# lixilinx/psgd_tf

Measured on AMD Instinct MI355X. Metric: uvd_update_apply_params_per_sec, higher is better.
Workload: dtype f32

## Files before the change

### psgd_tf_amd/csrc/psgd_uvd.hip

```cpp
#include "uvd_kernels.h"
#include "psgd_hip.h"
#include <math.h>

namespace psgd {

const UvdOps* uvd_ops_group0(int r);
const UvdOps* uvd_ops_group1(int r);
const UvdOps* uvd_ops_group2(int r);
const UvdOps* uvd_ops_group3(int r);

const UvdWideOps* uvd_wide_group0(int r);
const UvdWideOps* uvd_wide_group1(int r);
const UvdWideOps* uvd_wide_group2(int r);
const UvdWideOps* uvd_wide_group3(int r);
const UvdWideOps* uvd_wide_ops_for_rank(int r) {
  if (r <= PSGD_UVD_MAX_RANK || r > 2 * PSGD_UVD_MAX_RANK) return nullptr;
  switch ((r - 33) / 8) {
    case 0: return uvd_wide_group0(r);
    case 1: return uvd_wide_group1(r);
    case 2: return uvd_wide_group2(r);
    default: return uvd_wide_group3(r);
  }
}

// ... 44 lines not shown

static int ws_open(void* ws, int64_t ws_bytes, int64_t N, int r, Ws* out) {
  if (N <= 0) return PSGD_ERR_BAD_ARG;
  if (r < 1 || r > PSGD_UVD_MAX_RANK) return PSGD_ERR_RANK;
  if (!ws || (reinterpret_cast<uintptr_t>(ws) & 255)) return PSGD_ERR_WORKSPACE;
  const WsLayout L = ws_layout(N, r);
  if (ws_bytes < L.total) return PSGD_ERR_WORKSPACE;
  char* b = static_cast<char*>(ws);
  out->sums = reinterpret_cast<double*>(b + L.sums_off);
  out->coef = reinterpret_cast<float*>(b + L.coef_off);
  out->maxbuf = reinterpret_cast<float*>(b + L.max_off);
  out->part = b + L.part_off;
  out->pmax = reinterpret_cast<float*>(b + L.pmax_off);
  out->nabla = reinterpret_cast<float*>(b + L.nabla_off);
  return PSGD_OK;
}

static inline bool misaligned16(const void* p) { return (reinterpret_cast<uintptr_t>(p) & 15) != 0; }

static int g_tune_staging = 0;
static int g_tune_blocks_per_cu = 0;
static int g_tune_tiles_per_wave = 8;

constexpr int kProfSlots = 8;
constexpr int kProfMaxPairs = 4096;
struct ProfPair { hipEvent_t e0, e1; };
static int g_prof_on = 0;
static ProfPair g_prof_pairs[kProfSlots][kProfMaxPairs];
static int g_prof_created[kProfSlots];
static int g_prof_used[kProfSlots];

struct ProfScope {
  hipEvent_t e1 = nullptr;
  hipStream_t st;
  ProfScope(int slot, hipStream_t s) : st(s) {
    if (!g_prof_on || slot < 0 || slot >= kProfSlots || g_prof_used[slot] >= kProfMaxPairs) return;
    const int i = g_prof_used[slot];
    if (i >= g_prof_created[slot]) {
      if (hipEventCreate(&g_prof_pairs[slot][i].e0) != hipSuccess) return;
      if (hipEventCreate(&g_prof_pairs[slot][i].e1) != hipSuccess) return;
      g_prof_created[slot] = i + 1;
    }
    g_prof_used[slot] = i + 1;
    (void)hipEventRecord(g_prof_pairs[slot][i].e0, st);
    e1 = g_prof_pairs[slot][i].e1;
  }
  ~ProfScope() {
    if (e1) (void)hipEventRecord(e1, st);
  }
};

static int num_cus() {
  static int n = 0;
  if (n == 0) {
    int dev = 0;
    (void)hipGetDevice(&dev);
    int v = 0;
    if (hipDeviceGetAttribute(&v, hipDeviceAttributeMultiprocessorCount, dev) != hipSuccess || v <= 0) v = 256;
    n = v;
  }
  return n;
}

static inline int use_nt(int64_t N, int r) {
  if (g_tune_staging == 1) return 0;
  if (g_tune_staging == 2) return 1;
  return (int64_t)N * r * 8 > (int64_t)192 * 1024 * 1024;
}

int policy_nt(int64_t stream_bytes) {
  if (g_tune_staging == 1) return 0;
  if (g_tune_staging == 2) return 1;
  return stream_bytes > (int64_t)192 * 1024 * 1024;
}
int policy_grid_blocks(int occ) {
  if (occ <= 0) occ = 1;
  if (g_tune_blocks_per_cu > 0 && g_tune_blocks_per_cu < occ) occ = g_tune_blocks_per_cu;
  if (g_tune_blocks_per_cu < 0) occ = -g_tune_blocks_per_cu;
  return occ;
}
int device_cus() { return num_cus(); }

static int g_tune_grid[16] = {0};

static int sweep_grid(const UvdOps* ops, int r, int which, int64_t N, int hard_cap) {
  static int occ_cache[PSGD_UVD_MAX_RANK + 1][16];
  if (which >= 0 && which < 16 && g_tune_grid[which] > 0) {
    const int64_t tiles = (N + ops->tile_rows - 1) / ops->tile_rows;
    int64_t grid = (tiles + kWavesPerBlock - 1) / kWavesPerBlock;
    if (grid > g_tune_grid[which]) grid = g_tune_grid[which];
    if (grid > hard_cap) grid = hard_cap;
    return (int)(grid < 1 ? 1 : grid);
  }
  int occ = occ_cache[r][which];
  if (occ == 0) {
    occ = ops->occupancy(which);
    if (occ <= 0) occ = 1;
    occ_cache[r][which] = occ;
  }
  if (which == kOccUpdS2U || which == kOccUpdS2V || which == kOccUpdS2F) {
    const int want = ((long)ops->tile_rows * r * 4 >= 4096) ? 1 : 2;
    if (want < occ) occ = want;
  } else if (which == kOccFinal) {
    occ = 1;
  }
  if (g_tune_blocks_per_cu > 0 && g_tune_blocks_per_cu < occ) occ = g_tune_blocks_per_cu;
  if (g_tune_blocks_per_cu < 0) occ = -g_tune_blocks_per_cu;
  const int64_t tiles = (N + ops->tile_rows - 1) / ops->tile_rows;
  int64_t grid = (tiles + kWavesPerBlock - 1) / kWavesPerBlock;
  int64_t cap = (int64_t)num_cus() * occ;
  if (g_tune_blocks_per_cu == 0) {
    int64_t want = tiles / (kWavesPerBlock * (g_tune_tiles_per_wave > 0 ? g_tune_tiles_per_wave : 1));
    if (want < num_cus()) want = num_cus();
    if (cap > want) cap = want;
  }
  if (grid > cap) grid = cap;
  if (grid > hard_cap) grid = hard_cap;
  if (grid < 1) grid = 1;
  return (int)grid;
}

template <class T>
__global__ __launch_bounds__(kThreads) void k_reduce_sum(const T* __restrict__ part, int G, int L,
                                                         double* __restrict__ sums, float* __restrict__ coef) {
  __shared__ double red[kWavesPerBlock][64];
  const int lane = threadIdx.x & 63, w = threadIdx.x >> 6;
  const int id = blockIdx.x * 64 + lane;
  double s = 0.0;
  if (id < L) {
    int b = w;
    for (; b + 7 * kWavesPerBlock < G; b += 8 * kWavesPerBlock) {
      T x[8];
#pragma unroll
      for (int u = 0; u < 8; ++u) x[u] = part[(long)(b + u * kWavesPerBlock) * L + id];
#pragma unroll
      for (int u = 0; u < 8; ++u) s += (double)x[u];
    }
    for (; b < G; b += kWavesPerBlock) s += (double)part[(long)b * L + id];
  }
  red[w][lane] = s;
  __syncthreads();
  if (w == 0 && id < L) {
    const double t = ((red[0][lane] + red[1][lane]) + red[2][lane]) + red[3][lane];
    sums[id] = t;
    if (coef) coef[id] = (float)t;
  }
}

__global__ __launch_bounds__(kThreads) void k_reduce_sum_t(const float* __restrict__ part, int G, int L,
                                                           double* __restrict__ sums, float* __restrict__ coef) {
  const int lane = threadIdx.x & 63;
  const int id = blockIdx.x * kWavesPerBlock + (threadIdx.x >> 6);
  if (id >= L) return;
  const float* p = part + (long)id * G;
  float x[kMaxGrid / 64];
#pragma unroll
  for (int u = 0; u < kMaxGrid / 64; ++u) x[u] = p[min(lane + 64 * u, G - 1)];
  double s = 0.0;
#pragma unroll
  for (int u = 0; u < kMaxGrid / 64; ++u) s += (lane + 64 * u < G) ? (double)x[u] : 0.0;
#pragma unroll
  for (int off = 32; off > 0; off >>= 1) s += __shfl_down(s, off, 64);
  if (lane == 0) {
    sums[id] = s;
    if (coef) coef[id] = (float)s;
  }
// ... 653 lines not shown
      for (int off = 32; off > 0; off >>= 1) sum += __shfl_down(sum, off, 64);
      if (lane == 0) { pqs[e] = sum; pq[e] = sum; }
    }
  } else {
    for (int e = tid; e < 4 * r; e += blockDim.x) pqs[e] = pq[e];
    if (tid == 0) mx = maxbuf[0];
  }
  const int nb = (2 * r + 2 + 15) / 16;
  auto Gm = [&](int a, int b) -> double {
    if constexpr (DENSE) return gram[a * (2 * r + 2) + b];
    if (a > b) { const int t = a; a = b; b = t; }
    const int bi = a >> 4, bj = b >> 4, i = a & 15, j = b & 15;
    const int p = bi * nb - (bi * (bi - 1)) / 2 + (bj - bi);
    return gram[p * 256 + (i & 3) * 64 + (((i >> 2) << 4) | j)];
  };
  const bool act = tid < r;
  if (act) {
    for (int j0 = 0; j0 < r; j0 += 8) {
      double t[8];
#pragma unroll
      for (int u = 0; u < 8; ++u) t[u] = Gm(tid, (j0 + u < r) ? j0 + u : 0);
#pragma unroll
      for (int u = 0; u < 8; ++u)
        if (j0 + u < r) A[tid][j0 + u] = t[u];
    }
    if (update_U) {
      const double mu = c64[4 * r], aa = c64[4 * r + 1], ab = c64[4 * r + 2], bb = c64[4 * r + 3];
      const double Ua = c64[tid], Ub = c64[r + tid], c1 = c64[2 * r + tid], c2 = c64[3 * r + tid];
      for (int j = 0; j < r; ++j) {
        const double Uaj = c64[j], Ubj = c64[r + j], c1j = c64[2 * r + j], c2j = c64[3 * r + j];
        A[tid][j] += -mu * (Ua * c1j + c1 * Uaj - Ub * c2j - c2 * Ubj) +
                     mu * mu * (aa * c1 * c1j - ab * (c1 * c2j + c2 * c1j) + bb * c2 * c2j);
      }
    }
  }
  __syncthreads();
  const double mud = (double)(step / (mx + tiny));
  if (act) s1n[tid] = pqs[r + tid] - mud * pqs[3 * r + tid];
  __syncthreads();
  if (act) {
    double s2 = pqs[tid] - mud * pqs[2 * r + tid];
    for (int k = 0; k < r; ++k) s2 += A[tid][k] * s1n[k];
    coef[tid] = (float)s1n[tid];
    coef[r + tid] = (float)s2;
    s_out[tid] = s1n[tid];
    s_out[r + tid] = s2;
  }
}

}

using namespace psgd;

#define PSGD_CHECK_LAUNCH(expr)                 \
  do {                                          \
    const int _e = (expr);                      \
    if (_e != 0) return PSGD_ERR_LAUNCH;        \
  } while (0)

static inline int last_launch() { return (int)hipGetLastError(); }

extern "C" {

int psgd_abi_version(void) { return PSGD_ABI_VERSION; }

const char* psgd_error_string(int code) {
  switch (code) {
    case PSGD_OK: return "ok";
    case PSGD_ERR_BAD_ARG: return "bad argument (null pointer or non-positive size)";
    case PSGD_ERR_RANK: return "rank of modification outside [1, 32]";
    case PSGD_ERR_WORKSPACE: return "workspace missing, too small or not 256-byte aligned";
    case PSGD_ERR_ALIGN: return "matrix pointer not 16-byte aligned";
    case PSGD_ERR_LAUNCH: return "HIP kernel launch failed";
    case PSGD_ERR_SHAPE: return "inconsistent or unsupported matrix shapes";
    default: return "unknown error";
  }
}

int psgd_set_tuning(int key, int value) {
  if (key == 0) { g_tune_staging = value; return PSGD_OK; }
  if (key == 1) { g_tune_blocks_per_cu = value; return PSGD_OK; }
  if (key == 2) { g_tune_coef = value; return PSGD_OK; }
  if (key == 3) { g_tune_tiles_per_wave = value; return PSGD_OK; }
  if (key >= 10 && key < 26) { g_tune_grid[key - 10] = value; return PSGD_OK; }
  return PSGD_ERR_BAD_ARG;
}

int psgd_prof_enable(int on) {
  g_prof_on = on ? 1 : 0;
  for (int s = 0; s < kProfSlots; ++s) g_prof_used[s] = 0;
  return PSGD_OK;
}

int psgd_prof_collect(int slot, double* total_ms, int* count) {
  if (slot < 0 || slot >= kProfSlots || !total_ms || !count) return PSGD_ERR_BAD_ARG;
  double tot = 0.0;
  int n = 0;
  for (int i = 0; i < g_prof_used[slot]; ++i) {
    float ms = 0.0f;
    if (hipEventSynchronize(g_prof_pairs[slot][i].e1) != hipSuccess) continue;
    if (hipEventElapsedTime(&ms, g_prof_pairs[slot][i].e0, g_prof_pairs[slot][i].e1) != hipSuccess) continue;
    tot += ms;
    ++n;
  }
  g_prof_used[slot] = 0;
  *total_ms = tot;
  *count = n;
  return PSGD_OK;
}

int64_t psgd_uvd_workspace_bytes(int64_t N, int r) {
  if (N <= 0) return PSGD_ERR_BAD_ARG;
  if (r < 1 || r > PSGD_UVD_MAX_RANK) return PSGD_ERR_RANK;
  return ws_layout(N, r).total;
}

int psgd_uvd_ws_region(int which, int stage, int64_t N, int r, int64_t* offset_bytes, int64_t* count) {
  if (!offset_bytes || !count || N <= 0) return PSGD_ERR_BAD_ARG;
  if (r < 1 || r > PSGD_UVD_MAX_RANK) return PSGD_ERR_RANK;
  const WsLayout L = ws_layout(N, r);
  const int nc = 2 * r + 2, nb = (nc + 15) / 16, np = nb * (nb + 1) / 2;
  if (which == PSGD_WS_SUMS_F64) {
    if (stage == 1) { *offset_bytes = L.sums_off; *count = r; return PSGD_OK; }
    if (stage == 2) { *offset_bytes = L.sums_off + (int64_t)r * 8; *count = r; return PSGD_OK; }
    if (stage == 11) { *offset_bytes = L.sums_off; *count = (int64_t)np * 256; return PSGD_OK; }
    if (stage == 13) { *offset_bytes = L.sums_off + (int64_t)kPqSumsOff * 8; *count = 4 * r; return PSGD_OK; }
  } else if (which == PSGD_WS_MAX_F32) {
    if (stage == 10) { *offset_bytes = L.max_off; *count = 2; return PSGD_OK; }
    if (stage == 12) { *offset_bytes = L.max_off + 8; *count = 1; return PSGD_OK; }
  } else if (which == PSGD_WS_SEND_F64) {
    if (stage == 1 || stage == 2 || stage == 11) return psgd_uvd_ws_region(PSGD_WS_SUMS_F64, stage, N, r, offset_bytes, count);
    if (stage == 10) { *offset_bytes = L.sums_off + (int64_t)kBalD64Off * 8; *count = 2; return PSGD_OK; }
    if (stage == 12) { *offset_bytes = L.sums_off + (int64_t)(kPqSumsOff + 4 * r) * 8; *count = 1; return PSGD_OK; }
    if (stage == 13) { *offset_bytes = L.sums_off + (int64_t)kPqSumsOff * 8; *count = 4 * r + 1; return PSGD_OK; }
  }
  return PSGD_ERR_BAD_ARG;
}

int psgd_uvd_fold_gathered_f64(int stage, const double* gathered, int world, int64_t N, int r, void* ws,
                               int64_t ws_bytes, void* stream) {
  if (!gathered || world < 1) return PSGD_ERR_BAD_ARG;
  Ws w;
  const int rc = ws_open(ws, ws_bytes, N, r, &w);
  if (rc) return rc;
  int64_t off = 0, count = 0;
  const int rr = psgd_uvd_ws_region(PSGD_WS_SEND_F64, stage, N, r, &off, &count);
  if (rr) return rr;
  double* dst = reinterpret_cast<double*>(static_cast<char*>(ws) + off);
  int nsum = (int)count;
  float* maxdst = nullptr;
  if (stage == 10) { nsum = 0; maxdst = w.maxbuf; }
  else if (stage == 12) { nsum = 0; maxdst = w.maxbuf + 2; }
  else if (stage == 13) { nsum = 4 * r; maxdst = w.maxbuf + 2; }
  hipLaunchKernelGGL(k_fold_gathered, dim3(((int)count + 255) / 256), dim3(256), 0, static_cast<hipStream_t>(stream),
                     gathered, world, (int)count, nsum, dst, maxdst);
  PSGD_CHECK_LAUNCH(last_launch());
  return PSGD_OK;
}

int psgd_uvd_apply_sweep1_f32(const float* V, const float* d, const float* g, int64_t N, int r, void* ws,
                              int64_t ws_bytes, void* stream) {
  if (!V || !d || !g) return PSGD_ERR_BAD_ARG;
  Ws w;
  const int rc = ws_open(ws, ws_bytes, N, r, &w);
  if (rc) return rc;
  if (misaligned16(V)) return PSGD_ERR_ALIGN;
// ... 688 lines not shown
```

### psgd_tf_amd/csrc/uvd_kernels.h

```cpp
#pragma once
#include <hip/hip_runtime.h>
#include <stdint.h>
#include <type_traits>
#include "nanmax.h"

namespace psgd {

constexpr int kWave = 64;
constexpr int kWavesPerBlock = 4;
constexpr int kThreads = kWave * kWavesPerBlock;
constexpr int kMaxGrid = 2048;
constexpr int kGramMaxGrid = 1024;
#ifndef PSGD_TILE_CHUNK
#define PSGD_TILE_CHUNK 1
#endif
constexpr int kTileChunk = PSGD_TILE_CHUNK;

typedef float f32x4 __attribute__((ext_vector_type(4)));

#ifndef PSGD_WAVE_ID_VGPR
__device__ __forceinline__ int wave_in_block() { return __builtin_amdgcn_readfirstlane((int)(threadIdx.x >> 6)); }
#else
__device__ __forceinline__ int wave_in_block() { return (int)(threadIdx.x >> 6); }
#endif
// ... 862 lines not shown
    sweep_rows<R, 2, NV, (UPDATE_U ? 0 : 1), NT>(mats, vecs, UPDATE_U ? U : V, N, lds, body);
  }
  block_max_store(vmax, red, part_max + blockIdx.x);
}

template <int R, bool NT>
__global__ __launch_bounds__(kThreads) void k_uvd_final(const float* U, const float* V, float* d, const float* nabla,
                                                        const float* g, float* out, long N,
                                                        const float* __restrict__ coef, const float* __restrict__ maxbuf,
                                                        float step, float tiny) {
  __shared__ __attribute__((aligned(16))) float lds[kWavesPerBlock][sweep_lds_floats<R, 2, 3>()];
  const float mu = step / (maxbuf[0] + tiny);
  const float* const mats[2] = {U, V};
  const float* const vecs[3] = {d, nabla, g};
  sweep_rows<R, 2, 3, -1, NT>(mats, vecs, nullptr, N, lds[wave_in_block()],
                              [&](long row, bool valid, float (&x)[2][R], float (&s)[3]) {
                                const float dn = s[0] - (mu * s[0]) * s[1];
                                const float g1 = dn * s[2] + dot_row<R>(x[0], coef);
                                const float o = dn * (g1 + dot_row<R>(x[1], coef + R));
                                if (valid) {
                                  stream_store<NT>(d + row, dn);
                                  stream_store<NT>(out + row, o);
                                }
                              });
}

template <int R, bool NT, bool STR = false>
__global__ __launch_bounds__(kThreads) void k_rank2_update(float* M, const float* a, const float* b, long N,
                                                           const float* __restrict__ coef, long ld = R) {
  __shared__ __attribute__((aligned(16))) float lds[kWavesPerBlock][sweep_lds_floats<R, 1, 2>()];
  const float* const mats[1] = {M};
  const float* const vecs[2] = {a, b};
  sweep_rows<R, 1, 2, 0, NT, STR>(mats, vecs, M, N, lds[wave_in_block()],
                                  [&](long, bool, float (&x)[1][R], float (&s)[2]) {
#pragma unroll
                                    for (int c = 0; c < R; ++c) x[0][c] = x[0][c] - (s[0] * coef[c] - s[1] * coef[R + c]);
                                  }, NoTileHook(), RowStrides{{ld, ld}});
}

struct UvdOps {
  int tile_rows;
  int gram_len;
  int (*colreduce)(int nt, int nvec, const float* M, const float* a, const float* b, long N, float* part, int grid, hipStream_t st);
  int (*apply_s2)(int nt, const float* U, const float* d, const float* g, float* g1out, long N, const float* coef, float* part, int grid, hipStream_t st);
  int (*apply_s3)(int nt, const float* V, const float* d, float* out, long N, const float* coef, int grid, hipStream_t st);
  int (*rowdot_axpy)(int nt, const float* M, const float* x, float* out, long N, const float* coef, int grid, hipStream_t st);
  int (*update_gram)(int nt, const float* U, const float* V, const float* d, const float* v, const float* h, long N, double* part, int grid, hipStream_t st);
  int (*update_s2)(int nt, int update_U, float* U, float* V, const float* d, const float* v, const float* h, const float* g, long N, const float* coef, float* nabla, float* part_max, double* part_pq, int grid, hipStream_t st);
  int (*colreduce4)(int nt, const float* M, const float* const* x, long N, double* part, int grid, hipStream_t st);
  int (*rowdot_axpy4)(int nt, const float* M, const float* const* x, float* const* o, int ncols, long N, const float* coef, int grid, hipStream_t st);
  int (*rank2_update)(int nt, float* M, const float* a, const float* b, long N, const float* coef, int grid, hipStream_t st);
  int (*final_sweep)(int nt, const float* U, const float* V, float* d, const float* nabla, const float* g, float* out, long N, const float* coef, const float* maxbuf, float step, float tiny, int grid, hipStream_t st);
  int (*apply4_s1)(int nt, const float* V, const float* d, const float* const* x, long N, double* part, int grid, hipStream_t st);
  int (*apply4_s2)(int nt, const float* U, const float* d, const float* const* x, float* const* o, int ncols, long N, const float* coef, double* part, int grid, hipStream_t st);
  int (*apply4_s3)(int nt, const float* V, const float* d, float* const* o, int ncols, long N, const float* coef, int grid, hipStream_t st);
  int load_vec;
  int (*update_gram_ld)(const float* U, long ldU, const float* V, long ldV, const float* d, const float* v, const float* h, long N, double* part, int grid, hipStream_t st);
  int (*colreduce4_ld)(const float* M, long ld, const float* const* x, long N, double* part, int grid, hipStream_t st);
  int (*rowdot_axpy4_ld)(const float* M, long ld, const float* const* x, float* const* o, int ncols, long N, const float* coef, int grid, hipStream_t st);
  int (*rank2_update_ld)(float* M, long ld, const float* a, const float* b, long N, const float* coef, int grid, hipStream_t st);
  int (*occupancy)(int which);
};

struct UvdWideOps {
  int tile_rows;
  int (*colreduce4)(int nt, const float* M, const float* const* x, long N, double* part, int grid, hipStream_t st);
  int (*rowdot_axpy4)(int nt, const float* M, const float* const* x, float* const* o, int ncols, long N, const float* coef, int grid, hipStream_t st);
  int (*rank2_update)(int nt, float* M, const float* a, const float* b, long N, const float* coef, int grid, hipStream_t st);
  int (*apply4_s1)(int nt, const float* V, const float* d, const float* const* x, long N, double* part, int grid, hipStream_t st);
  int (*apply4_s2)(int nt, const float* U, const float* d, const float* const* x, float* const* o, int ncols, long N, const float* coef, double* part, int grid, hipStream_t st);
  int (*apply4_s3)(int nt, const float* V, const float* d, float* const* o, int ncols, long N, const float* coef, int grid, hipStream_t st);
  int (*update_s2)(int nt, int update_U, float* U, float* V, const float* d, const float* v, const float* h, const float* g, long N, const float* coef, float* nabla, float* part_max, double* part_pq, int grid, hipStream_t st);
  int (*final_sweep)(int nt, const float* U, const float* V, float* d, const float* nabla, const float* g, float* out, long N, const float* coef, const float* maxbuf, float step, float tiny, int grid, hipStream_t st);
};
const UvdWideOps* uvd_wide_ops_for_rank(int r);

enum { kOccColreduce = 0, kOccApplyS2, kOccApplyS3, kOccRowdot, kOccGram, kOccUpdS2U, kOccUpdS2V, kOccUpdS2F, kOccFinal };

const UvdOps* uvd_ops_for_rank(int r);

int policy_nt(int64_t stream_bytes);
int policy_grid_blocks(int occupancy);
int device_cus();

}
```

### psgd_tf_amd/csrc/uvd_wide_gram.hip

```cpp
#include "uvd_kernels.h"

#include "psgd_hip.h"

#include <cstdlib>

namespace psgd {

#ifndef GW_ACC64_LDS
#define GW_ACC64_LDS 0
#endif
#ifndef GW_DBG
#define GW_DBG 0
#endif
constexpr int kGwRows = 32;
constexpr int kGwThreads = 1024;
constexpr int kGwMulWaves = 11;
constexpr int kGwDepth = 4;

__host__ __device__ constexpr int gw_pair_index(int NB, int bi, int bj) { return bi * NB - (bi * (bi - 1)) / 2 + (bj - bi); }

struct GwPlan {
  int owner[15];
  int slot0[15];
  int max_load;
  int base[kGwMulWaves];
  int load[kGwMulWaves];
};
template <int NB>
constexpr GwPlan gw_make_plan() {
  constexpr int NS = (NB + 1) / 2, NSP = NS * (NS + 1) / 2;
  GwPlan p{};
  int load[kGwMulWaves] = {};
  int wt[15] = {};
  bool placed[15] = {};
  for (int si = 0; si < NS; ++si)
    for (int sj = si; sj < NS; ++sj) {
      const int na = (NB - 2 * si) < 2 ? (NB - 2 * si) : 2, nb = (NB - 2 * sj) < 2 ? (NB - 2 * sj) : 2;
      wt[gw_pair_index(NS, si, sj)] = si == sj ? na * (na + 1) / 2 : na * nb;
    }
  for (int round = 0; round < NSP; ++round) {
    int best = -1;
    for (int sp = 0; sp < NSP; ++sp)
      if (!placed[sp] && (best < 0 || wt[sp] > wt[best])) best = sp;
    int w = 0;
    for (int k = 1; k < kGwMulWaves; ++k)
      if (load[k] < load[w]) w = k;
    p.owner[best] = w;
    p.slot0[best] = load[w];
    load[w] += wt[best];
    placed[best] = true;
  }
  for (int k = 0; k < kGwMulWaves; ++k)
    if (load[k] > p.max_load) p.max_load = load[k];
  for (int k = 0, b = 0; k < kGwMulWaves; ++k) { p.base[k] = b; p.load[k] = load[k]; b += load[k]; }
  return p;
}
template <int NB> struct GwPlanOf { static constexpr GwPlan value = gw_make_plan<NB>(); };

template <int N> struct GwInt { static constexpr int value = N; };
template <int I, int N, class F>
__device__ __forceinline__ void gw_static_for(F&& f) {
  if constexpr (I < N) {
    f(GwInt<I>{});
    gw_static_for<I + 1, N>(f);
  }
}

#ifndef GW_UNIT_COLMAJOR
template <int NC> __device__ __forceinline__ int gw_unit(int col, int rg) { return rg * NC + col; }
#else
template <int NC> __device__ __forceinline__ int gw_unit(int col, int rg) { return col * 4 + (rg ^ ((col >> 2) & 2)); }
#endif

template <int NB, bool NT, bool TAIL>
__global__ __launch_bounds__(kGwThreads) void k_gram_wide(const float* __restrict__ U, const float* __restrict__ V,
                                                          const float* __restrict__ d, const float* __restrict__ v,
                                                          const float* __restrict__ h, long N, int r, long ntiles, long tile0,
                                                          double* __restrict__ part) {
  constexpr int NC = NB * 16;
  constexpr int NPW = GwPlanOf<NB>::value.max_load;
  constexpr int NP = NB * (NB + 1) / 2;
  typedef unsigned int u32x4g __attribute__((ext_vector_type(4)));
  __shared__ __attribute__((aligned(16))) u32x4g PL[2][3][NC * 4 + 16];
#if GW_ACC64_LDS
  __shared__ double A64[NP][4][64];
#endif
  const int tid = threadIdx.x, lane = tid & 63, wave = tid >> 6;
  const long G = gridDim.x;
  const long tfirst = TAIL ? tile0 : (long)blockIdx.x;
  if (TAIL) ntiles = tile0 + 1;

  const long nmine = (ntiles - tfirst + G - 1) / G;
  const long tlast = tfirst + (nmine - 1) * G;
  auto clampt = [&](long t) { return t < tlast ? t : tlast; };
  auto tile_loop = [&](auto&& prologue, auto&& step) {
    __syncthreads();
    prologue();
    __syncthreads();
    for (long i = 0; i < nmine; i += kGwDepth)
      gw_static_for<0, kGwDepth>([&](auto ic) {
        step(ic, tfirst + (i + decltype(ic)::value) * G);
        __syncthreads();
      });
  };
  if (wave < 4) {
    const int col = tid % r, g0 = tid / r;
    const bool on = g0 < 4;
    const unsigned e0 = on ? (unsigned)(g0 * 8 * r + col) : 0u;
    const unsigned eb0 = e0 * 4u;
    const int un0 = gw_unit<NC>(col, on ? g0 : 0), un1 = gw_unit<NC>(r + col, on ? g0 : 0);
    for (int i = tid; i < 2 * 3 * (NC * 4 + 16); i += 256) (&PL[0][0][0])[i] = u32x4g{0u, 0u, 0u, 0u};
    float px[kGwDepth][16];
    auto fetch = [&](long t, auto ic) {
      constexpr int ib = decltype(ic)::value;
      if constexpr (!TAIL) {
        const long toff0 = t * kGwRows * r;
        const long toff = ((long)__builtin_amdgcn_readfirstlane((int)(toff0 >> 32)) << 32) |
                          (unsigned)__builtin_amdgcn_readfirstlane((int)toff0);
        const unsigned tbytes = (unsigned)(kGwRows * r * 4);
        const auto ru = __builtin_amdgcn_make_buffer_rsrc(const_cast<float*>(U + toff), 0, tbytes, 0x00020000);
        const auto rv = __builtin_amdgcn_make_buffer_rsrc(const_cast<float*>(V + toff), 0, tbytes, 0x00020000);
        constexpr int aux = NT ? 2 : 0;
#pragma unroll
        for (int j = 0; j < 8; ++j) {
          px[ib][j] = __builtin_bit_cast(float, __builtin_amdgcn_raw_buffer_load_b32(ru, eb0, j * r * 4, aux));
          px[ib][8 + j] = __builtin_bit_cast(float, __builtin_amdgcn_raw_buffer_load_b32(rv, eb0, j * r * 4, aux));
        }
      } else {
        const long row0 = t * kGwRows + (on ? g0 : 0) * 8;
#pragma unroll
        for (int j = 0; j < 8; ++j) {
          const long row = row0 + j, rc = (row < N ? row : N - 1) * r + col;
          const float xu = stream_load<NT>(U + rc), xv = stream_load<NT>(V + rc);
          px[ib][j] = (on && row < N) ? xu : 0.0f;
          px[ib][8 + j] = (on && row < N) ? xv : 0.0f;
        }
      }
    };
    auto split_to = [&](int buf, auto ic) {
      constexpr int ib = decltype(ic)::value;
      if (GW_DBG & 4) {
#pragma unroll
        for (int j = 0; j < 16; ++j) asm volatile("" ::"v"(px[ib][j]));
        return;
      }
      if (!on) return;
      bf16x8 fh, fm, fl;
      float x[8];
#pragma unroll
      for (int hh = 0; hh < 2; ++hh) {
#pragma unroll
        for (int j = 0; j < 8; ++j) x[j] = px[ib][hh * 8 + j];
        split3_bf16(x, fh, fm, fl);
        const int un = hh ? un1 : un0;
        PL[buf][0][un] = __builtin_bit_cast(u32x4g, fh);
        PL[buf][1][un] = __builtin_bit_cast(u32x4g, fm);
        PL[buf][2][un] = __builtin_bit_cast(u32x4g, fl);
      }
    };
    const long t0 = tfirst;
    tile_loop(
        [&]() {
          gw_static_for<0, kGwDepth>([&](auto ic) { fetch(clampt(t0 + decltype(ic)::value * G), ic); });
          split_to(0, GwInt<0>{});
          fetch(clampt(t0 + kGwDepth * G), GwInt<0>{});
        },
        [&](auto ic, long t) {
          constexpr int q = decltype(ic)::value, slot = (q + 1) % kGwDepth;
          split_to((q + 1) & 1, GwInt<slot>{});
          fetch(clampt(t + (1 + kGwDepth) * G), GwInt<slot>{});
        });
    return;
  }
  if (wave == 4) {
    float* TW = reinterpret_cast<float*>(&PL[1][2][NC * 4]);
    const int tw_un = gw_unit<NC>(2 * r + (lane & 1), (lane >> 1) & 3);
    float pd[kGwDepth], ph[kGwDepth], pv[kGwDepth];
    bool pok[kGwDepth];
    const int it = lane >> 3;
    auto fetch = [&](long t, auto ic) {
      const long row = t * kGwRows + (it >> 1) * 8 + (lane & 7), rc = (!TAIL || row < N) ? row : N - 1;
      pd[decltype(ic)::value] = d[rc];
      ph[decltype(ic)::value] = h[rc];
      pv[decltype(ic)::value] = v[rc];
      pok[decltype(ic)::value] = !TAIL || row < N;
    };
    auto split_to = [&](int b, auto ic) {
      const float dd = pd[decltype(ic)::value], hh = ph[decltype(ic)::value], vv = pv[decltype(ic)::value];
      if (GW_DBG & 8) {
        asm volatile("" ::"v"(dd), "v"(hh), "v"(vv));
        return;
      }
      const float val = (it & 1) ? vv / dd : dd * hh;
      TW[lane] = pok[decltype(ic)::value] ? val : 0.0f;
      asm volatile("s_waitcnt lgkmcnt(0)" ::: "memory");
      __builtin_amdgcn_wave_barrier();
      if (lane < 8) {
        float x[8];
#pragma unroll
        for (int j = 0; j < 8; ++j) x[j] = TW[lane * 8 + j];
        bf16x8 fh, fm, fl;
        split3_bf16(x, fh, fm, fl);
        PL[b][0][tw_un] = __builtin_bit_cast(u32x4g, fh);
        PL[b][1][tw_un] = __builtin_bit_cast(u32x4g, fm);
        PL[b][2][tw_un] = __builtin_bit_cast(u32x4g, fl);
      }
      asm volatile("s_waitcnt lgkmcnt(0)" ::: "memory");
      __builtin_amdgcn_wave_barrier();
    };
    const long t0 = tfirst;
    tile_loop(
        [&]() {
          gw_static_for<0, kGwDepth>([&](auto ic) { fetch(clampt(t0 + decltype(ic)::value * G), ic); });
          split_to(0, GwInt<0>{});
          fetch(clampt(t0 + kGwDepth * G), GwInt<0>{});
        },
        [&](auto ic, long t) {
          constexpr int q = decltype(ic)::value, slot = (q + 1) % kGwDepth;
          split_to((q + 1) & 1, GwInt<slot>{});
          fetch(clampt(t + (1 + kGwDepth) * G), GwInt<slot>{});
        });
    return;
  }
  const int mw = wave - 5;
  f32x4 acc[NPW];
#if GW_ACC64_LDS
  int my_base = 0, my_load = 0;
  gw_static_for<0, kGwMulWaves>([&](auto kc) {
    if (mw == decltype(kc)::value) { my_base = GwPlanOf<NB>::value.base[decltype(kc)::value]; my_load = GwPlanOf<NB>::value.load[decltype(kc)::value]; }
  });
  double (*my64)[4][64] = A64 + my_base;
#pragma unroll
  for (int p = 0; p < NPW; ++p) {
    acc[p] = f32x4{0.f, 0.f, 0.f, 0.f};
    if (p < my_load)
#pragma unroll
      for (int e = 0; e < 4; ++e) my64[p][e][lane] = 0.0;
  }
  auto fold = [&]() {
#pragma unroll
    for (int p = 0; p < NPW; ++p) {
      if (p < my_load)
#pragma unroll
        for (int e = 0; e < 4; ++e) my64[p][e][lane] += (double)acc[p][e];
      acc[p] = f32x4{0.f, 0.f, 0.f, 0.f};
    }
  };
#else
  double acc64[NPW][4];
#pragma unroll
  for (int p = 0; p < NPW; ++p) {
    acc[p] = f32x4{0.f, 0.f, 0.f, 0.f};
#pragma unroll
    for (int e = 0; e < 4; ++e) acc64[p][e] = 0.0;
  }
  auto fold = [&]() {
#pragma unroll
    for (int p = 0; p < NPW; ++p) {
#pragma unroll
      for (int e = 0; e < 4; ++e) acc64[p][e] += (double)acc[p][e];
      acc[p] = f32x4{0.f, 0.f, 0.f, 0.f};
    }
  };
#endif
  int since = 0;
  tile_loop([]() {}, [&](auto ic, long t) {
    if (t >= ntiles) return;
    const int buf = decltype(ic)::value & 1;
    auto frag = [&](int b, bf16x8 (&f)[3]) {
      const int un = gw_unit<NC>(b * 16 + (lane & 15), lane >> 4);
#pragma unroll
      for (int pl = 0; pl < 3; ++pl) f[pl] = __builtin_bit_cast(bf16x8, PL[buf][pl][un]);
    };
    constexpr int NS = (NB + 1) / 2;
    gw_static_for<0, NS>([&](auto sic) {
      constexpr int si = decltype(sic)::value;
      gw_static_for<si, NS>([&](auto sjc) {
        constexpr int sj = decltype(sjc)::value;
        constexpr int sp = gw_pair_index(NS, si, sj);
        constexpr int own = GwPlanOf<NB>::value.owner[sp], s0 = GwPlanOf<NB>::value.slot0[sp];
        constexpr int na = (NB - 2 * si) < 2 ? (NB - 2 * si) : 2, nb = (NB - 2 * sj) < 2 ? (NB - 2 * sj) : 2;
        if (mw == own && !(GW_DBG & 2)) {
          bf16x8 fa[2][3], fb[2][3];
          gw_static_for<0, nb>([&](auto c) { frag(2 * sj + decltype(c)::value, fb[decltype(c)::value]); });
          if constexpr (si != sj) gw_static_for<0, na>([&](auto c) { frag(2 * si + decltype(c)::value, fa[decltype(c)::value]); });
          gw_static_for<0, 6>([&](auto tc) {
            constexpr int term = decltype(tc)::value;
            constexpr int pa = term == 0 ? 1 : term == 1 ? 0 : term == 2 ? 2 : term == 3 ? 0 : term == 4 ? 1 : 0;
            constexpr int pb = term == 0 ? 1 : term == 1 ? 2 : term == 2 ? 0 : term == 3 ? 1 : term == 4 ? 0 : 0;
            gw_static_for<0, na>([&](auto ac) {
              constexpr int a = decltype(ac)::value;
              gw_static_for<(si == sj ? a : 0), nb>([&](auto bc) {
                constexpr int b = decltype(bc)::value;
                constexpr int slot = s0 + (si == sj ? (a == 0 ? b : nb + (b - 1)) : a * nb + b);
                if constexpr (si == sj) acc[slot] = __builtin_amdgcn_mfma_f32_16x16x32_bf16(fb[a][pa], fb[b][pb], acc[slot], 0, 0, 0);
                else acc[slot] = __builtin_amdgcn_mfma_f32_16x16x32_bf16(fa[a][pa], fb[b][pb], acc[slot], 0, 0, 0);
              });
            });
          });
        }
      });
    });
    if (++since == 256 / kGwRows) {
      fold();
      since = 0;
    }
  });
  fold();
  double* dst = part + (long)blockIdx.x * NP * 256;
  {
    constexpr int NS = (NB + 1) / 2;
    gw_static_for<0, NS>([&](auto sic) {
      constexpr int si = decltype(sic)::value;
      gw_static_for<si, NS>([&](auto sjc) {
        constexpr int sj = decltype(sjc)::value;
        constexpr int sp = gw_pair_index(NS, si, sj);
        constexpr int own = GwPlanOf<NB>::value.owner[sp], s0 = GwPlanOf<NB>::value.slot0[sp];
        constexpr int na = (NB - 2 * si) < 2 ? (NB - 2 * si) : 2, nb = (NB - 2 * sj) < 2 ? (NB - 2 * sj) : 2;
        if (mw == own) {
          gw_static_for<0, na>([&](auto ac) {
            constexpr int a = decltype(ac)::value;
            gw_static_for<(si == sj ? a : 0), nb>([&](auto bc) {
              constexpr int b = decltype(bc)::value;
              constexpr int slot = s0 + (si == sj ? (a == 0 ? b : nb + (b - 1)) : a * nb + b);
              constexpr int pi = gw_pair_index(NB, 2 * si + a, 2 * sj + b);
#pragma unroll
#if GW_ACC64_LDS
              for (int e = 0; e < 4; ++e) dst[pi * 256 + e * 64 + lane] = my64[slot][e][lane];
#else
              for (int e = 0; e < 4; ++e) dst[pi * 256 + e * 64 + lane] = acc64[slot][e];
#endif
            });
          });
        }
      });
    });
  }
}

__global__ __launch_bounds__(kThreads) void k_gram_wide_finish(const double* __restrict__ part, int nblocks, int NB, int ncol,
                                                               double* __restrict__ G) {
  const int NP = NB * (NB + 1) / 2;
  const int idx = blockIdx.x * kThreads + threadIdx.x;
  if (idx >= NP * 256) return;
  const int p = idx >> 8, q = idx & 255, e = q >> 6, l = q & 63;
  int bi = 0, rem = p;
  while (rem >= NB - bi) { rem -= NB - bi; ++bi; }
  const int bj = bi + rem;
  double s = 0.0;
  const double* src = part + (long)p * 256 + q;
  const long st = (long)NP * 256;
  int b = 0;
  for (; b + 8 <= nblocks; b += 8) {
    double x[8];
#pragma unroll
    for (int u = 0; u < 8; ++u) x[u] = src[(b + u) * st];
#pragma unroll
    for (int u = 0; u < 8; ++u) s += x[u];
  }
  for (; b < nblocks; ++b) s += src[b * st];
  const int i = 16 * bi + 4 * (l >> 4) + e, j = 16 * bj + (l & 15);
  if (i < ncol && j < ncol && (bi != bj || i <= j)) {
    G[(long)i * ncol + j] = s;
    G[(long)j * ncol + i] = s;
  }
}

template <int NB>
static int launch_gram_wide(int nt, const float* U, const float* V, const float* d, const float* v, const float* h, long N, int r,
                            double* part, int grid, hipStream_t st) {
  const long nfull = N / kGwRows;
  if (nfull > 0) {
    if (nt) hipLaunchKernelGGL((k_gram_wide<NB, true, false>), dim3(grid), dim3(kGwThreads), 0, st, U, V, d, v, h, N, r, nfull, 0L, part);
    else hipLaunchKernelGGL((k_gram_wide<NB, false, false>), dim3(grid), dim3(kGwThreads), 0, st, U, V, d, v, h, N, r, nfull, 0L, part);
    if (hipGetLastError() != hipSuccess) return 1;
  }
  if (N % kGwRows) {
    double* tail = part + (long)(nfull > 0 ? grid : 0) * (NB * (NB + 1) / 2) * 256;
    hipLaunchKernelGGL((k_gram_wide<NB, false, true>), dim3(1), dim3(kGwThreads), 0, st, U, V, d, v, h, N, r, nfull + 1, nfull, tail);
  }
  return (int)hipGetLastError();
}

}

using namespace psgd;

static int gram_wide_grid(int64_t N) {
  const int64_t tiles = N / kGwRows;
  int64_t g = (int64_t)device_cus();
  if (g > tiles) g = tiles;
  if (g < 1) g = 1;
  return (int)g;
}

extern "C" {

int64_t psgd_uvd_gram_wide_scratch_bytes(int64_t N, int r) {
  if (N <= 0 || r <= PSGD_UVD_MAX_RANK || r > 2 * PSGD_UVD_MAX_RANK) return PSGD_ERR_RANK;
  const int NB = (2 * r + 2 + 15) / 16;
  return (int64_t)(gram_wide_grid(N) + 1) * (NB * (NB + 1) / 2) * 256 * 8;
}

int psgd_uvd_gram_wide_f32(const float* U, const float* V, const float* d, const float* v, const float* h, int64_t N, int r,
                           double* G, void* scratch, int64_t scratch_bytes, void* stream) {
  if (!U || !V || !d || !v || !h || !G || N <= 0) return PSGD_ERR_BAD_ARG;
  if (r <= PSGD_UVD_MAX_RANK || r > 2 * PSGD_UVD_MAX_RANK) return PSGD_ERR_RANK;
  const int64_t need = psgd_uvd_gram_wide_scratch_bytes(N, r);
  if (!scratch || (reinterpret_cast<uintptr_t>(scratch) & 255) || scratch_bytes < need) return PSGD_ERR_WORKSPACE;
  hipStream_t st = static_cast<hipStream_t>(stream);
  const int NB = (2 * r + 2 + 15) / 16, grid = gram_wide_grid(N);
  static const int env_nt = getenv("PSGD_GW_NT") ? atoi(getenv("PSGD_GW_NT")) : -1;
  const int nt = env_nt >= 0 ? env_nt : policy_nt(2 * N * r * 4);
  double* part = static_cast<double*>(scratch);
  int e = 1;
  switch (NB) {
    case 5: e = launch_gram_wide<5>(nt, U, V, d, v, h, N, r, part, grid, st); break;
    case 6: e = launch_gram_wide<6>(nt, U, V, d, v, h, N, r, part, grid, st); break;
    case 7: e = launch_gram_wide<7>(nt, U, V, d, v, h, N, r, part, grid, st); break;
    case 8: e = launch_gram_wide<8>(nt, U, V, d, v, h, N, r, part, grid, st); break;
    case 9: e = launch_gram_wide<9>(nt, U, V, d, v, h, N, r, part, grid, st); break;
    default: return PSGD_ERR_RANK;
  }
  if (e) return PSGD_ERR_LAUNCH;
  const int NP = NB * (NB + 1) / 2, ncol = 2 * r + 2;
  const int nsets = (N / kGwRows > 0 ? grid : 0) + (N % kGwRows ? 1 : 0);
  hipLaunchKernelGGL(k_gram_wide_finish, dim3((NP * 256 + kThreads - 1) / kThreads), dim3(kThreads), 0, st, part, nsets, NB, ncol, G);
  return hipGetLastError() == hipSuccess ? PSGD_OK : PSGD_ERR_LAUNCH;
}

}
```

Measured before the change: 9.482 billion.

## Use a four-stage LDS ring in the wide Gram kernel with register-prefetched fragments

Result: slower. 9.088 billion (-4.2%).

```diff
diff --git a/psgd_tf_amd/csrc/psgd_uvd.hip b/psgd_tf_amd/csrc/psgd_uvd.hip
--- a/psgd_tf_amd/csrc/psgd_uvd.hip
+++ b/psgd_tf_amd/csrc/psgd_uvd.hip
@@ -150,6 +150,9 @@
 int device_cus() { return num_cus(); }
 
 static int g_tune_grid[16] = {0};
+static int g_tune_gram_wide = 0;
+int policy_grid_cap(int which) { return which >= 0 && which < 16 && g_tune_grid[which] > 0 ? g_tune_grid[which] : 0; }
+int policy_gram_wide_two_buffers() { return g_tune_gram_wide == 1; }
 
 static int sweep_grid(const UvdOps* ops, int r, int which, int64_t N, int hard_cap) {
   static int occ_cache[PSGD_UVD_MAX_RANK + 1][16];
@@ -969,6 +972,7 @@
   if (key == 1) { g_tune_blocks_per_cu = value; return PSGD_OK; }
   if (key == 2) { g_tune_coef = value; return PSGD_OK; }
   if (key == 3) { g_tune_tiles_per_wave = value; return PSGD_OK; }
+  if (key == 4) { g_tune_gram_wide = value; return PSGD_OK; }
   if (key >= 10 && key < 26) { g_tune_grid[key - 10] = value; return PSGD_OK; }
   return PSGD_ERR_BAD_ARG;
 }
diff --git a/psgd_tf_amd/csrc/uvd_kernels.h b/psgd_tf_amd/csrc/uvd_kernels.h
--- a/psgd_tf_amd/csrc/uvd_kernels.h
+++ b/psgd_tf_amd/csrc/uvd_kernels.h
@@ -968,5 +968,7 @@
 int policy_nt(int64_t stream_bytes);
 int policy_grid_blocks(int occupancy);
 int device_cus();
-
-}
+int policy_grid_cap(int which);
+int policy_gram_wide_two_buffers();
+
+}
diff --git a/psgd_tf_amd/csrc/uvd_wide_gram.hip b/psgd_tf_amd/csrc/uvd_wide_gram.hip
--- a/psgd_tf_amd/csrc/uvd_wide_gram.hip
+++ b/psgd_tf_amd/csrc/uvd_wide_gram.hip
@@ -16,6 +16,7 @@
 constexpr int kGwThreads = 1024;
 constexpr int kGwMulWaves = 11;
 constexpr int kGwDepth = 4;
+constexpr int kGwStages = 4;
 
 __host__ __device__ constexpr int gw_pair_index(int NB, int bi, int bj) { return bi * NB - (bi * (bi - 1)) / 2 + (bj - bi); }
 
@@ -25,6 +26,8 @@
   int max_load;
   int base[kGwMulWaves];
   int load[kGwMulWaves];
+  int dsi[kGwMulWaves];
+  int dsj[kGwMulWaves];
 };
 template <int NB>
 constexpr GwPlan gw_make_plan() {
@@ -52,7 +55,12 @@
   }
   for (int k = 0; k < kGwMulWaves; ++k)
     if (load[k] > p.max_load) p.max_load = load[k];
-  for (int k = 0, b = 0; k < kGwMulWaves; ++k) { p.base[k] = b; p.load[k] = load[k]; b += load[k]; }
+  for (int k = 0, b = 0; k < kGwMulWaves; ++k) { p.base[k] = b; p.load[k] = load[k]; b += load[k]; p.dsi[k] = -1; p.dsj[k] = -1; }
+  for (int si = 0; si < NS; ++si)
+    for (int sj = si + 1; sj < NS; ++sj) {
+      const int sp = gw_pair_index(NS, si, sj), w = p.owner[sp];
+      if (NB - 2 * sj >= 2 && load[w] == 4) { p.dsi[w] = si; p.dsj[w] = sj; }
+    }
   return p;
 }
 template <int NB> struct GwPlanOf { static constexpr GwPlan value = gw_make_plan<NB>(); };
@@ -72,7 +80,7 @@
 template <int NC> __device__ __forceinline__ int gw_unit(int col, int rg) { return col * 4 + (rg ^ ((col >> 2) & 2)); }
 #endif
 
-template <int NB, bool NT, bool TAIL>
+template <int NB, bool NT, bool TAIL, bool RING>
 __global__ __launch_bounds__(kGwThreads) void k_gram_wide(const float* __restrict__ U, const float* __restrict__ V,
                                                           const float* __restrict__ d, const float* __restrict__ v,
                                                           const float* __restrict__ h, long N, int r, long ntiles, long tile0,
@@ -81,7 +89,10 @@
   constexpr int NPW = GwPlanOf<NB>::value.max_load;
   constexpr int NP = NB * (NB + 1) / 2;
   typedef unsigned int u32x4g __attribute__((ext_vector_type(4)));
-  __shared__ __attribute__((aligned(16))) u32x4g PL[2][3][NC * 4 + 16];
+  constexpr int NST = RING ? kGwStages : 2;
+  constexpr int AHEAD = RING ? 2 : 1;
+  static_assert(kGwStages == kGwDepth, "a tile's stage is its ordinal mod the unroll of the tile loop");
+  __shared__ __attribute__((aligned(16))) u32x4g PL[NST][3][NC * 4 + 16];
 #if GW_ACC64_LDS
   __shared__ double A64[NP][4][64];
 #endif
@@ -93,10 +104,14 @@
   const long nmine = (ntiles - tfirst + G - 1) / G;
   const long tlast = tfirst + (nmine - 1) * G;
   auto clampt = [&](long t) { return t < tlast ? t : tlast; };
-  auto tile_loop = [&](auto&& prologue, auto&& step) {
+  auto tile_loop = [&](auto&& prologue, auto&& second, auto&& step) {
     __syncthreads();
     prologue();
     __syncthreads();
+    if constexpr (RING) {
+      second();
+      __syncthreads();
+    }
     for (long i = 0; i < nmine; i += kGwDepth)
       gw_static_for<0, kGwDepth>([&](auto ic) {
         step(ic, tfirst + (i + decltype(ic)::value) * G);
@@ -109,7 +124,7 @@
     const unsigned e0 = on ? (unsigned)(g0 * 8 * r + col) : 0u;
     const unsigned eb0 = e0 * 4u;
     const int un0 = gw_unit<NC>(col, on ? g0 : 0), un1 = gw_unit<NC>(r + col, on ? g0 : 0);
-    for (int i = tid; i < 2 * 3 * (NC * 4 + 16); i += 256) (&PL[0][0][0])[i] = u32x4g{0u, 0u, 0u, 0u};
+    for (int i = tid; i < NST * 3 * (NC * 4 + 16); i += 256) (&PL[0][0][0])[i] = u32x4g{0u, 0u, 0u, 0u};
     float px[kGwDepth][16];
     auto fetch = [&](long t, auto ic) {
       constexpr int ib = decltype(ic)::value;
@@ -165,10 +180,14 @@
           split_to(0, GwInt<0>{});
           fetch(clampt(t0 + kGwDepth * G), GwInt<0>{});
         },
+        [&]() {
+          split_to(1, GwInt<1>{});
+          fetch(clampt(t0 + (1 + kGwDepth) * G), GwInt<1>{});
+        },
         [&](auto ic, long t) {
-          constexpr int q = decltype(ic)::value, slot = (q + 1) % kGwDepth;
-          split_to((q + 1) & 1, GwInt<slot>{});
-          fetch(clampt(t + (1 + kGwDepth) * G), GwInt<slot>{});
+          constexpr int q = decltype(ic)::value, slot = (q + AHEAD) % kGwDepth;
+          split_to((q + AHEAD) % NST, GwInt<slot>{});
+          fetch(clampt(t + (AHEAD + kGwDepth) * G), GwInt<slot>{});
         });
     return;
   }
@@ -215,10 +234,14 @@
           split_to(0, GwInt<0>{});
           fetch(clampt(t0 + kGwDepth * G), GwInt<0>{});
         },
+        [&]() {
+          split_to(1, GwInt<1>{});
+          fetch(clampt(t0 + (1 + kGwDepth) * G), GwInt<1>{});
+        },
         [&](auto ic, long t) {
-          constexpr int q = decltype(ic)::value, slot = (q + 1) % kGwDepth;
-          split_to((q + 1) & 1, GwInt<slot>{});
-          fetch(clampt(t + (1 + kGwDepth) * G), GwInt<slot>{});
+          constexpr int q = decltype(ic)::value, slot = (q + AHEAD) % kGwDepth;
+          split_to((q + AHEAD) % NST, GwInt<slot>{});
+          fetch(clampt(t + (AHEAD + kGwDepth) * G), GwInt<slot>{});
         });
     return;
   }
@@ -264,9 +287,49 @@
   };
 #endif
   int since = 0;
-  tile_loop([]() {}, [&](auto ic, long t) {
+  int dsi = -1, dsj = -1;
+  if constexpr (RING)
+    gw_static_for<0, kGwMulWaves>([&](auto kc) {
+      if (mw == decltype(kc)::value) { dsi = GwPlanOf<NB>::value.dsi[decltype(kc)::value]; dsj = GwPlanOf<NB>::value.dsj[decltype(kc)::value]; }
+    });
+  if (RING && dsi >= 0) {
+    bf16x8 fa[2][3], fb[2][3];
+    const int una = gw_unit<NC>(2 * dsi * 16 + (lane & 15), lane >> 4), unb = gw_unit<NC>(2 * dsj * 16 + (lane & 15), lane >> 4);
+    auto read_stage = [&](auto sc) {
+      constexpr int stg = decltype(sc)::value;
+#pragma unroll
+      for (int c = 0; c < 2; ++c)
+#pragma unroll
+        for (int pl = 0; pl < 3; ++pl) {
+          fa[c][pl] = __builtin_bit_cast(bf16x8, PL[stg][pl][una + c * 16]);
+          fb[c][pl] = __builtin_bit_cast(bf16x8, PL[stg][pl][unb + c * 16]);
+        }
+    };
+    tile_loop([]() {}, [&]() { read_stage(GwInt<0>{}); },
+              [&](auto ic, long t) {
+                constexpr int q = decltype(ic)::value;
+                if (t < ntiles && !(GW_DBG & 2)) {
+                  gw_static_for<0, 6>([&](auto tc) {
+                    constexpr int term = decltype(tc)::value;
+                    constexpr int pa = term == 0 ? 1 : term == 1 ? 0 : term == 2 ? 2 : term == 3 ? 0 : term == 4 ? 1 : 0;
+                    constexpr int pb = term == 0 ? 1 : term == 1 ? 2 : term == 2 ? 0 : term == 3 ? 1 : term == 4 ? 0 : 0;
+#pragma unroll
+                    for (int a = 0; a < 2; ++a)
+#pragma unroll
+                      for (int b = 0; b < 2; ++b)
+                        acc[a * 2 + b] = __builtin_amdgcn_mfma_f32_16x16x32_bf16(fa[a][pa], fb[b][pb], acc[a * 2 + b], 0, 0, 0);
+                  });
+                  if (++since == 256 / kGwRows) {
+                    fold();
+                    since = 0;
+                  }
+                }
+                read_stage(GwInt<(q + 1) % kGwStages>{});
+              });
+  } else
+  tile_loop([]() {}, []() {}, [&](auto ic, long t) {
     if (t >= ntiles) return;
-    const int buf = decltype(ic)::value & 1;
+    constexpr int buf = decltype(ic)::value % NST;
     auto frag = [&](int b, bf16x8 (&f)[3]) {
       const int un = gw_unit<NC>(b * 16 + (lane & 15), lane >> 4);
 #pragma unroll
@@ -367,17 +430,22 @@
 }
 
 template <int NB>
-static int launch_gram_wide(int nt, const float* U, const float* V, const float* d, const float* v, const float* h, long N, int r,
+static int launch_gram_wide(int ring, int nt, const float* U, const float* V, const float* d, const float* v, const float* h, long N, int r,
                             double* part, int grid, hipStream_t st) {
   const long nfull = N / kGwRows;
   if (nfull > 0) {
-    if (nt) hipLaunchKernelGGL((k_gram_wide<NB, true, false>), dim3(grid), dim3(kGwThreads), 0, st, U, V, d, v, h, N, r, nfull, 0L, part);
-    else hipLaunchKernelGGL((k_gram_wide<NB, false, false>), dim3(grid), dim3(kGwThreads), 0, st, U, V, d, v, h, N, r, nfull, 0L, part);
+    if (ring) {
+      if (nt) hipLaunchKernelGGL((k_gram_wide<NB, true, false, true>), dim3(grid), dim3(kGwThreads), 0, st, U, V, d, v, h, N, r, nfull, 0L, part);
+      else hipLaunchKernelGGL((k_gram_wide<NB, false, false, true>), dim3(grid), dim3(kGwThreads), 0, st, U, V, d, v, h, N, r, nfull, 0L, part);
+    } else {
+      if (nt) hipLaunchKernelGGL((k_gram_wide<NB, true, false, false>), dim3(grid), dim3(kGwThreads), 0, st, U, V, d, v, h, N, r, nfull, 0L, part);
+      else hipLaunchKernelGGL((k_gram_wide<NB, false, false, false>), dim3(grid), dim3(kGwThreads), 0, st, U, V, d, v, h, N, r, nfull, 0L, part);
+    }
     if (hipGetLastError() != hipSuccess) return 1;
   }
   if (N % kGwRows) {
     double* tail = part + (long)(nfull > 0 ? grid : 0) * (NB * (NB + 1) / 2) * 256;
-    hipLaunchKernelGGL((k_gram_wide<NB, false, true>), dim3(1), dim3(kGwThreads), 0, st, U, V, d, v, h, N, r, nfull + 1, nfull, tail);
+    hipLaunchKernelGGL((k_gram_wide<NB, false, true, false>), dim3(1), dim3(kGwThreads), 0, st, U, V, d, v, h, N, r, nfull + 1, nfull, tail);
   }
   return (int)hipGetLastError();
 }
@@ -389,6 +457,8 @@
 static int gram_wide_grid(int64_t N) {
   const int64_t tiles = N / kGwRows;
   int64_t g = (int64_t)device_cus();
+  const int cap = policy_grid_cap(kOccGram);
+  if (cap > 0 && g > cap) g = cap;
   if (g > tiles) g = tiles;
   if (g < 1) g = 1;
   return (int)g;
@@ -413,13 +483,14 @@
   static const int env_nt = getenv("PSGD_GW_NT") ? atoi(getenv("PSGD_GW_NT")) : -1;
   const int nt = env_nt >= 0 ? env_nt : policy_nt(2 * N * r * 4);
   double* part = static_cast<double*>(scratch);
+  const int ring = policy_gram_wide_two_buffers() ? 0 : 1;
   int e = 1;
   switch (NB) {
-    case 5: e = launch_gram_wide<5>(nt, U, V, d, v, h, N, r, part, grid, st); break;
-    case 6: e = launch_gram_wide<6>(nt, U, V, d, v, h, N, r, part, grid, st); break;
-    case 7: e = launch_gram_wide<7>(nt, U, V, d, v, h, N, r, part, grid, st); break;
-    case 8: e = launch_gram_wide<8>(nt, U, V, d, v, h, N, r, part, grid, st); break;
-    case 9: e = launch_gram_wide<9>(nt, U, V, d, v, h, N, r, part, grid, st); break;
+    case 5: e = launch_gram_wide<5>(ring, nt, U, V, d, v, h, N, r, part, grid, st); break;
+    case 6: e = launch_gram_wide<6>(ring, nt, U, V, d, v, h, N, r, part, grid, st); break;
+    case 7: e = launch_gram_wide<7>(ring, nt, U, V, d, v, h, N, r, part, grid, st); break;
+    case 8: e = launch_gram_wide<8>(ring, nt, U, V, d, v, h, N, r, part, grid, st); break;
+    case 9: e = launch_gram_wide<9>(ring, nt, U, V, d, v, h, N, r, part, grid, st); break;
     default: return PSGD_ERR_RANK;
   }
   if (e) return PSGD_ERR_LAUNCH;
```
